# musyoku/chainer-speech-recognition

Hardware: AMD Instinct MI355X
Metric: utterances/sec (T=1000, 40x3 feat, |V|~3000) CTC train step (higher is better)
Workload: dtype bf16

## Files before the change

### chainer-speech-recognition_amd/asr/_lib.py

```python
import ctypes
import os

import torch

_HERE = os.path.dirname(os.path.abspath(__file__))
_ACT = os.environ.get("ASR_ACT", "").lower()
LIB_PATH = os.environ.get("ASR_HIP_LIB") or os.path.join(os.path.dirname(_HERE),
                                                        "libasr_hip_f16.so" if _ACT in ("f16", "fp16", "float16", "half") else "libasr_hip.so")

_lib = None


def act_dtype():
    return torch.float16 if lib().asr_act_dtype() else torch.bfloat16


def debug_flag(key, default):
    for item in os.environ.get("ASR_DEBUG", "").split(","):
        k, _, v = item.strip().partition("=")
        if k == key and v:
            return int(v)
    return default

c_void_p, c_int, c_float, c_size_t = ctypes.c_void_p, ctypes.c_int, ctypes.c_float, ctypes.c_size_t
c_double = ctypes.c_double
c_longlong = ctypes.c_longlong

SIGNATURES = {
    "asr_version": (c_int, []),
    "asr_act_dtype": (c_int, []),
    "asr_stream_delay": (c_int, [c_void_p, c_int]),
    "asr_occupy_cus": (c_int, [c_void_p, c_int, c_int, c_int]),
    "asr_stream_traffic": (c_int, [c_void_p, c_int, c_int, c_int, c_void_p, c_longlong]),
    "asr_ctc_workspace_bytes": (c_size_t, [c_int] * 5),
    "asr_ctc_forward": (c_int, [c_void_p] * 6 + [c_int] * 5 + [c_void_p] * 3 + [c_size_t]),
    "asr_ctc_forward_lse": (c_int, [c_void_p] * 6 + [c_int] * 5 + [c_void_p] * 3 + [c_size_t, c_void_p]),
    "asr_ctc_backward": (c_int, [c_void_p] * 3 + [c_int] * 5 + [c_void_p, c_int, c_float, c_void_p, c_void_p, c_size_t]),
    "asr_ctc_loss_grad": (c_int, [c_void_p] * 6 + [c_int] * 5 + [c_float] + [c_void_p] * 4 + [c_size_t]),
    "asr_ctc_nbest_workspace_bytes": (c_size_t, [c_int] * 5),
    "asr_ctc_nbest_forward": (c_int, [c_void_p] * 5 + [c_int] * 6 + [c_void_p, c_void_p, c_size_t]),
    "asr_ctc_nbest_backward": (c_int, [c_void_p] * 3 + [c_int] * 5 + [c_void_p] * 3 + [c_size_t]),
    "asr_gram_ctc_nbest_workspace_bytes": (c_size_t, [c_int] * 5),
    "asr_gram_ctc_nbest_forward": (c_int, [c_void_p] * 6 + [c_int] * 6 + [c_void_p, c_void_p, c_size_t]),
    "asr_gram_ctc_nbest_backward": (c_int, [c_void_p] * 3 + [c_int] * 5 + [c_void_p] * 3 + [c_size_t]),
    "asr_specgram": (c_int, [c_void_p, c_void_p, c_int, c_void_p, c_longlong] + [c_int] * 4 + [c_double, c_void_p, c_void_p, c_int,
                               c_void_p, c_void_p, c_int, c_void_p]),
    "asr_mel_bands_bytes": (c_size_t, []),
    "asr_mel_bands": (c_int, [c_void_p, c_void_p, c_int, c_int, c_void_p, c_size_t]),
    "asr_specgram_bands": (c_int, [c_void_p, c_void_p, c_int, c_void_p, c_longlong] + [c_int] * 4 + [c_double, c_void_p, c_void_p, c_int,
                                     c_void_p, c_void_p, c_int, c_void_p, c_void_p]),
    "asr_logmel": (c_int, [c_void_p] * 3 + [c_longlong, c_int, c_int, c_void_p]),
    "asr_deltas": (c_int, [c_void_p] * 3 + [c_int] * 4 + [c_void_p] * 3),
    "asr_batchnorm_stats": (c_int, [c_void_p, c_void_p, c_longlong, c_int, c_float, c_float] + [c_void_p] * 5),
    "asr_rsqrt_eps": (c_int, [c_void_p, c_void_p, c_float, c_void_p, c_int]),
    "asr_batchnorm_fwd": (c_int, [c_void_p] * 6 + [c_longlong, c_int, c_void_p]),
    "asr_batchnorm_bwd": (c_int, [c_void_p] * 6 + [c_longlong, c_int] + [c_void_p] * 4),
    "asr_cmn_pspec": (c_int, [c_void_p] * 3 + [c_int] * 3),
    "asr_add_white_noise": (c_int, [c_void_p] * 3 + [c_longlong, c_int, c_void_p, ctypes.c_ulonglong]),
    "asr_augment_specgram": (c_int, [c_void_p] * 5 + [c_int] * 4 + [c_void_p]),
    "asr_running_stats_update": (c_int, [c_void_p] * 3 + [c_int] * 3 + [c_longlong] + [c_void_p] * 4),
    "asr_normalize_bcmt": (c_int, [c_void_p] * 4 + [c_int] * 3),
    "asr_argmax_rows": (c_int, [c_void_p, c_void_p, c_int, c_int, c_int, c_void_p]),
    "asr_ctc_collapse": (c_int, [c_void_p] * 3 + [c_int] * 4 + [c_void_p] * 2),
    "asr_edit_distance": (c_int, [c_void_p, c_void_p, c_void_p, c_int, c_void_p, c_void_p, c_int, c_int, c_void_p]),
    "asr_edit_align_workspace_bytes": (c_size_t, [c_int] * 3),
    "asr_edit_align": (c_int, [c_void_p, c_void_p, c_void_p, c_int, c_void_p, c_void_p, c_int, c_int] + [c_void_p] * 4 + [c_size_t]),
    "asr_nbest_pairwise_distance": (c_int, [c_void_p] * 3 + [c_int] * 3 + [c_void_p]),
    "asr_nbest_consensus_workspace_bytes": (c_size_t, [c_int] * 3),
    "asr_nbest_consensus": (c_int, [c_void_p] * 5 + [c_int] * 3 + [c_void_p, c_void_p, c_size_t]),
    "asr_ctc_beam_workspace_bytes": (c_size_t, [c_int] * 5),
    "asr_ctc_beam_search": (c_int, [c_void_p] * 3 + [c_int] * 6 + [c_float, c_void_p, c_size_t] + [c_void_p] * 3),
    "asr_ngram_score": (c_int, [c_void_p] * 2 + [c_int, c_void_p, c_void_p] + [c_int] * 3 + [c_void_p] * 2 + [c_int] * 4 + [c_void_p] * 2),
    "asr_ctc_beam_lm_workspace_bytes": (c_size_t, [c_int] * 5),
    "asr_ctc_beam_search_lm": (c_int, [c_void_p] * 3 + [c_int] * 6 + [c_float, c_void_p, c_int, c_void_p, c_void_p] + [c_int] * 5
                               + [c_float, c_float, c_void_p, c_size_t] + [c_void_p] * 5),
    "asr_ctx_score": (c_int, [c_void_p] * 3 + [c_int] * 2 + [c_void_p] + [c_int] * 2 + [c_void_p] * 2 + [c_int] * 3 + [c_void_p] * 2),
    "asr_ctc_beam_bias_workspace_bytes": (c_size_t, [c_int] * 5),
    "asr_ctc_beam_search_bias": (c_int, [c_void_p] * 3 + [c_int] * 6 + [c_float, c_void_p, c_int, c_void_p, c_void_p] + [c_int] * 5
                                 + [c_float, c_float, c_void_p, c_size_t] + [c_void_p] * 7 + [c_int] * 2 + [c_void_p, c_int, c_void_p]),
    "asr_ctc_beam_stream_state_bytes": (c_size_t, [c_int] * 5),
    "asr_ctc_beam_stream_workspace_bytes": (c_size_t, [c_int] * 5),
    "asr_ctc_beam_stream_reset": (c_int, [c_void_p] * 2 + [c_size_t] + [c_int] * 6 + [c_void_p]),
    "asr_ctc_beam_stream_advance": (c_int, [c_void_p] * 3 + [c_int] * 6 + [c_float, c_void_p, c_int, c_void_p, c_void_p] + [c_int] * 3
                                    + [c_void_p] * 2 + [c_int] * 2 + [c_void_p, c_int, c_float, c_float, c_int, c_int]
                                    + [c_void_p, c_size_t] * 2),
    "asr_ctc_beam_stream_result": (c_int, [c_void_p] * 2 + [c_int, c_void_p, c_void_p] + [c_int] * 3 + [c_void_p] * 2 + [c_int] * 2
                                   + [c_void_p, c_int, c_float, c_float] + [c_int] * 6 + [c_void_p, c_size_t] + [c_void_p] * 7),
    "asr_gram_ctc_beam_workspace_bytes": (c_size_t, [c_int] * 5),
    "asr_gram_ctc_beam_search": (c_int, [c_void_p] * 3 + [c_int] * 6 + [c_float, c_void_p, c_void_p, c_size_t] + [c_void_p] * 3),
    "asr_gram_ctc_beam_lm_workspace_bytes": (c_size_t, [c_int] * 5),
    "asr_gram_ctc_beam_search_lm": (c_int, [c_void_p] * 3 + [c_int] * 6 + [c_float, c_void_p, c_void_p, c_int, c_void_p, c_void_p]
                                    + [c_int] * 5 + [c_float, c_float, c_void_p, c_size_t] + [c_void_p] * 5),
    "asr_gram_ctc_beam_stream_state_bytes": (c_size_t, [c_int] * 4),
    "asr_gram_ctc_beam_stream_workspace_bytes": (c_size_t, [c_int] * 5),
    "asr_gram_ctc_beam_stream_reset": (c_int, [c_void_p] * 2 + [c_size_t] + [c_int] * 4 + [c_void_p]),
    "asr_gram_ctc_beam_stream_advance": (c_int, [c_void_p] * 3 + [c_int] * 6 + [c_float, c_void_p, c_void_p, c_int, c_void_p, c_void_p]
                                         + [c_int] * 4 + [c_float, c_float, c_int, c_int] + [c_void_p, c_size_t] * 2),
    "asr_gram_ctc_beam_stream_result": (c_int, [c_void_p] * 2 + [c_int, c_void_p, c_void_p] + [c_int] * 5 + [c_float, c_float]
                                        + [c_int] * 5 + [c_void_p, c_size_t] + [c_void_p] * 6),
    "asr_gram_ctc_beam_bias_workspace_bytes": (c_size_t, [c_int] * 5),
    "asr_gram_ctc_beam_search_bias": (c_int, [c_void_p] * 3 + [c_int] * 6 + [c_float, c_void_p, c_void_p, c_int, c_void_p, c_void_p]
                                      + [c_int] * 5 + [c_float, c_float, c_void_p, c_size_t] + [c_void_p] * 7 + [c_int] * 2
                                      + [c_void_p, c_int, c_void_p]),
    "asr_gram_ctc_beam_bias_stream_state_bytes": (c_size_t, [c_int] * 5),
    "asr_gram_ctc_beam_bias_stream_reset": (c_int, [c_void_p] * 2 + [c_size_t] + [c_int] * 5 + [c_void_p]),
    "asr_gram_ctc_beam_bias_stream_advance": (c_int, [c_void_p] * 3 + [c_int] * 6 + [c_float, c_void_p, c_void_p, c_int, c_void_p,
                                                      c_void_p] + [c_int] * 4 + [c_void_p] * 2 + [c_int] * 2 + [c_void_p, c_int]
                                              + [c_float, c_float, c_int, c_int] + [c_void_p, c_size_t] * 2),
    "asr_gram_ctc_beam_bias_stream_result": (c_int, [c_void_p] * 2 + [c_int, c_void_p, c_void_p] + [c_int] * 5 + [c_void_p] * 2
                                             + [c_int] * 2 + [c_void_p, c_int] + [c_float, c_float] + [c_int] * 5
                                             + [c_void_p, c_size_t] + [c_void_p] * 7),
    "asr_ctc_align_workspace_bytes": (c_size_t, [c_int] * 5),
    "asr_ctc_align": (c_int, [c_void_p] * 6 + [c_int] * 5 + [c_void_p] * 9 + [c_size_t]),
    "asr_kws_workspace_bytes": (c_size_t, [c_int] * 3),
    "asr_kws_state_bytes": (c_size_t, [c_int] * 3),
    "asr_kws_state_reset": (c_int, [c_void_p] * 2 + [c_int] * 3 + [c_void_p]),
    "asr_kws_detect": (c_int, [c_void_p] * 3 + [c_int] * 4 + [c_void_p, c_int, c_void_p, c_void_p, c_int, c_int] + [c_void_p] * 5
                       + [c_size_t]),
    "asr_kws_hits": (c_int, [c_void_p] * 5 + [c_int] * 4 + [c_float] + [c_void_p] * 5),
# ... 147 lines not shown
```

### chainer-speech-recognition_amd/csrc/ctc.hip

```cpp
#include "common.hpp"
#include "ctc_ws.hpp"
#include "ctc_lattice.hpp"
#include "ctc_sweep.hpp"
#include "../../include/asr_hip.h"

namespace asr {
namespace ctc {

__global__ __launch_bounds__(256) void rows_kernel(const float* __restrict__ xs, const int* __restrict__ x_len,
                                                   const int* __restrict__ path_label, int T, int B, int V, int Sp,
                                                   float* __restrict__ lse_out, float* __restrict__ lp, const float* __restrict__ lse_in) {
    __shared__ float scratch[32];
    if (lse_in) {
        const int row = blockIdx.x * 4 + (int)(threadIdx.x >> 6), lane = threadIdx.x & 63;
        if (row >= T * B) return;
        const int t = row / B, b = row - t * B;
        const int xl = x_len ? min(x_len[b], T) : T;
        if (t >= xl) return;
        const float* x = xs + (size_t)row * V;
        const float lse = lse_in[row];
        if (lane == 0) lse_out[row] = lse;
        const int* pl = path_label + (size_t)b * Sp;
        float* out = lp + ((size_t)b * T + t) * Sp;
        for (int s = lane; s < Sp; s += 64) {
            const int l = pl[s];
            out[s] = l >= 0 ? x[l] - lse : -INFINITY;
        }
        return;
    }
    const int row = blockIdx.x;
    const int t = row / B, b = row - t * B;
    const int xl = x_len ? min(x_len[b], T) : T;
    if (t >= xl) return;
    const float* x = xs + (size_t)row * V;
    float m = -INFINITY;
    const bool vec = ((V & 3) == 0) && ((((uintptr_t)x) & 15) == 0);
    if (vec) {
        const float4* x4 = reinterpret_cast<const float4*>(x);
        for (int i = threadIdx.x; i < (V >> 2); i += blockDim.x) {
            const float4 v = x4[i];
            m = fmaxf(m, fmaxf(fmaxf(v.x, v.y), fmaxf(v.z, v.w)));
        }
    } else {
        for (int i = threadIdx.x; i < V; i += blockDim.x) m = fmaxf(m, x[i]);
    }
    m = block_max(m, scratch);
    float sum = 0.f;
    if (vec) {
        const float4* x4 = reinterpret_cast<const float4*>(x);
        for (int i = threadIdx.x; i < (V >> 2); i += blockDim.x) {
            const float4 v = x4[i];
            sum += __expf(v.x - m) + __expf(v.y - m) + __expf(v.z - m) + __expf(v.w - m);
        }
    } else {
        for (int i = threadIdx.x; i < V; i += blockDim.x) sum += __expf(x[i] - m);
    }
    sum = block_sum(sum, scratch);
    const float lse = m + __logf(sum);
    if (threadIdx.x == 0) lse_out[row] = lse;
    const int* pl = path_label + (size_t)b * Sp;
    float* out = lp + ((size_t)b * T + t) * Sp;
    for (int s = threadIdx.x; s < Sp; s += blockDim.x) {
        const int l = pl[s];
        out[s] = l >= 0 ? x[l] - lse : -INFINITY;
    }
}

constexpr int kOccChunk = 8192;

__global__ __launch_bounds__(256) void grad_kernel(const float* __restrict__ xs, const int* __restrict__ x_len,
                                                   const int* __restrict__ path_label,
                                                   const int* __restrict__ path_len, const float* __restrict__ lse_in,
                                                   const double* __restrict__ alpha, const double* __restrict__ beta,
                                                   const double* __restrict__ total, const float* __restrict__ gy,
                                                   int gy_per_utt, float scale, int T, int B, int V, int Sp,
                                                   float* __restrict__ grad) {
    extern __shared__ __attribute__((aligned(16))) char smem[];
    float* occ = reinterpret_cast<float*>(smem);
    const int row = blockIdx.x;
    const int t = row / B, b = row - t * B;
    const int xl = x_len ? min(x_len[b], T) : T;
    float* g = grad + (size_t)row * V;
    const bool vec = ((V & 3) == 0) && ((((uintptr_t)g) & 15) == 0) && ((((uintptr_t)(xs + (size_t)row * V)) & 15) == 0);
    if (t >= xl) {
        if (vec) {
            float4* g4 = reinterpret_cast<float4*>(g);
            for (int i = threadIdx.x; i < (V >> 2); i += blockDim.x) g4[i] = make_float4(0.f, 0.f, 0.f, 0.f);
        } else {
            for (int i = threadIdx.x; i < V; i += blockDim.x) g[i] = 0.f;
        }
        return;
    }
    const float* x = xs + (size_t)row * V;
    const float lse = lse_in[row];
    const double tot = total[b];
    float sc = scale;
    if (gy) sc *= gy_per_utt ? gy[b] : gy[0];
    const int S = path_len[b];
    const int* pl = path_label + (size_t)b * Sp;
    const double* al = alpha + ((size_t)b * T + t) * Sp;
    const double* be = beta + ((size_t)b * T + t) * Sp;
    for (int v0 = 0; v0 < V; v0 += kOccChunk) {
        const int vn = min(kOccChunk, V - v0);
        for (int i = threadIdx.x; i < vn; i += blockDim.x) occ[i] = 0.f;
        __syncthreads();
        if (tot != -INFINITY) {
            for (int s = threadIdx.x; s < S; s += blockDim.x) {
                const int l = pl[s];
                if (l >= v0 && l < v0 + vn) {
                    const double e = al[s] + be[s] - tot;
                    if (e > -80.0) atomicAdd(&occ[l - v0], expf((float)e));
                }
            }
        }
        __syncthreads();
        if (vec) {
            const float4* x4 = reinterpret_cast<const float4*>(x + v0);
            const float4* o4 = reinterpret_cast<const float4*>(occ);
            float4* g4 = reinterpret_cast<float4*>(g + v0);
            for (int i = threadIdx.x; i < (vn >> 2); i += blockDim.x) {
                const float4 xv = x4[i];
                const float4 ov = o4[i];
                float4 r;
                r.x = (__expf(xv.x - lse) - ov.x) * sc;
                r.y = (__expf(xv.y - lse) - ov.y) * sc;
                r.z = (__expf(xv.z - lse) - ov.z) * sc;
                r.w = (__expf(xv.w - lse) - ov.w) * sc;
                g4[i] = r;
            }
        } else {
            for (int i = threadIdx.x; i < vn; i += blockDim.x) g[v0 + i] = (__expf(x[v0 + i] - lse) - occ[i]) * sc;
        }
        __syncthreads();
    }
}

__global__ void mean_kernel(const float* __restrict__ loss, int B, float* __restrict__ out) {
    __shared__ float scratch[32];
    float s = 0.f;
    for (int i = threadIdx.x; i < B; i += blockDim.x) s += loss[i];
    s = block_sum(s, scratch);
    if (threadIdx.x == 0) out[0] = s / (float)B;
}

}
}

using namespace asr;
using namespace asr::ctc;

extern "C" size_t asr_ctc_workspace_bytes(int T, int B, int V, int Lmax, int gram) {
    (void)V;
    if (T <= 0 || B <= 0 || Lmax <= 0) return 0;
    return carve(nullptr, T, B, Lmax, gram).bytes;
}

extern "C" int asr_ctc_forward_lse(void* stream_, const float* xs, const int32_t* label_unigram,
                                   const int32_t* label_bigram, const int32_t* x_len, const int32_t* l_len, int T, int B,
                                   int V, int Lmax, int blank, float* loss_per_utt, float* loss_mean, void* workspace,
                                   size_t workspace_bytes, const float* row_lse) {
    if (!xs || !label_unigram || !loss_per_utt || !workspace) return ASR_ERR_BAD_ARG;
    if (T <= 0 || B <= 0 || V <= 0 || Lmax <= 0 || blank < 0 || blank >= V) return ASR_ERR_BAD_ARG;
    const int gram = label_bigram != nullptr;
    Workspace w = carve(workspace, T, B, Lmax, gram);
    if (workspace_bytes < w.bytes) return ASR_ERR_WORKSPACE;
    const int Sp = path_pad(Lmax, gram);
    const size_t lds = sizeof(double) * 2 * (Sp + 16) + sizeof(int) * (Sp + 8);
    if (lds > 150 * 1024) return ASR_ERR_UNSUPPORTED;
    hipStream_t stream = (hipStream_t)stream_;
    if (gram)
        hipLaunchKernelGGL(prep_kernel<true>, dim3(B), dim3(256), 0, stream, label_unigram, label_bigram, l_len, Lmax, Sp,
                           V, blank, w.path_label, w.path_mask, w.path_len);
    else
        hipLaunchKernelGGL(prep_kernel<false>, dim3(B), dim3(256), 0, stream, label_unigram, label_bigram, l_len, Lmax,
                           Sp, V, blank, w.path_label, w.path_mask, w.path_len);
    ASR_LAUNCH_CHECK();
    hipLaunchKernelGGL(rows_kernel, dim3(row_lse ? (T * B + 3) / 4 : T * B), dim3(256), 0, stream, xs, x_len, w.path_label, T, B, V, Sp, w.lse, w.lp, row_lse);
    ASR_LAUNCH_CHECK();
    const int threads = Sp < 1024 ? Sp : 1024;
    if (gram) {
        if (lds > 48 * 1024)
            (void)hipFuncSetAttribute((const void*)lattice_kernel<7>, hipFuncAttributeMaxDynamicSharedMemorySize, (int)lds);
        hipLaunchKernelGGL(lattice_kernel<7>, dim3(B, 2), dim3(threads), lds, stream, w.lp, x_len, w.path_label,
                           w.path_mask, w.path_len, T, B, Sp, w.alpha, w.beta, w.total, loss_per_utt);
    } else {
        if (lds > 48 * 1024)
            (void)hipFuncSetAttribute((const void*)lattice_kernel<3>, hipFuncAttributeMaxDynamicSharedMemorySize, (int)lds);
        hipLaunchKernelGGL(lattice_kernel<3>, dim3(B, 2), dim3(threads), lds, stream, w.lp, x_len, w.path_label,
                           w.path_mask, w.path_len, T, B, Sp, w.alpha, w.beta, w.total, loss_per_utt);
    }
    ASR_LAUNCH_CHECK();
    if (loss_mean) {
        hipLaunchKernelGGL(mean_kernel, dim3(1), dim3(256), 0, stream, loss_per_utt, B, loss_mean);
        ASR_LAUNCH_CHECK();
    }
    return ASR_OK;
}

extern "C" int asr_ctc_forward(void* stream_, const float* xs, const int32_t* label_unigram,
                               const int32_t* label_bigram, const int32_t* x_len, const int32_t* l_len, int T, int B,
                               int V, int Lmax, int blank, float* loss_per_utt, float* loss_mean, void* workspace,
                               size_t workspace_bytes) {
    return asr_ctc_forward_lse(stream_, xs, label_unigram, label_bigram, x_len, l_len, T, B, V, Lmax, blank, loss_per_utt, loss_mean,
                               workspace, workspace_bytes, nullptr);
}

extern "C" int asr_ctc_backward(void* stream_, const float* xs, const int32_t* x_len, int T, int B, int V, int Lmax,
                                int gram, const float* gy, int gy_per_utt, float scale, float* grad,
                                const void* workspace, size_t workspace_bytes) {
    if (!xs || !grad || !workspace) return ASR_ERR_BAD_ARG;
    if (T <= 0 || B <= 0 || V <= 0 || Lmax <= 0) return ASR_ERR_BAD_ARG;
    Workspace w = carve(const_cast<void*>(workspace), T, B, Lmax, gram);
    if (workspace_bytes < w.bytes) return ASR_ERR_WORKSPACE;
    const int Sp = path_pad(Lmax, gram);
    const size_t lds = sizeof(float) * (size_t)(V < kOccChunk ? (int)align_up(V, 4) : kOccChunk);
    hipStream_t stream = (hipStream_t)stream_;
    hipLaunchKernelGGL(grad_kernel, dim3(T * B), dim3(256), lds, stream, xs, x_len, w.path_label, w.path_len, w.lse,
                       w.alpha, w.beta, w.total, gy, gy_per_utt, scale, T, B, V, Sp, grad);
    ASR_LAUNCH_CHECK();
    return ASR_OK;
}

extern "C" int asr_ctc_loss_grad(void* stream, const float* xs, const int32_t* label_unigram,
                                 const int32_t* label_bigram, const int32_t* x_len, const int32_t* l_len, int T, int B,
                                 int V, int Lmax, int blank, float scale, float* loss_per_utt, float* loss_mean,
                                 float* grad, void* workspace, size_t workspace_bytes) {
    int rc = asr_ctc_forward(stream, xs, label_unigram, label_bigram, x_len, l_len, T, B, V, Lmax, blank, loss_per_utt,
                             loss_mean, workspace, workspace_bytes);
    if (rc != ASR_OK) return rc;
    return asr_ctc_backward(stream, xs, x_len, T, B, V, Lmax, label_bigram != nullptr, nullptr, 0, scale, grad,
                            workspace, workspace_bytes);
}
```

### chainer-speech-recognition_amd/csrc/ctc_sweep.hpp

```cpp
#pragma once
#include "common.hpp"
#include "ctc_lattice.hpp"

namespace asr {
namespace ctc {

template <int NK>
__device__ __forceinline__ double lse_masked(const double* v, int mask) {
    float f[NK];
#pragma unroll
    for (int j = 0; j < NK; ++j) f[j] = (mask & (1 << j)) ? (float)v[j] : -INFINITY;
    float m32 = -1e30f;
#pragma unroll
    for (int j = 0; j < NK; ++j) m32 = __builtin_fmaxf(m32, f[j]);
    const double m = (double)m32;
    float acc = 0.f;
#pragma unroll
    for (int j = 0; j < NK; ++j) {
        const float e = __expf((float)(v[j] - m));
        acc += (mask & (1 << j)) ? e : 0.f;
    }
    return m + (double)(__builtin_amdgcn_logf(acc) * 0.69314718f);
}

template <int NK>
__global__ __launch_bounds__(1024) void lattice_kernel(const float* __restrict__ lp, const int* __restrict__ x_len,
                                                       const int* __restrict__ path_label,
                                                       const int* __restrict__ path_mask,
                                                       const int* __restrict__ path_len, int T, int B, int Sp,
                                                       double* __restrict__ alpha, double* __restrict__ beta,
                                                       double* __restrict__ total, float* __restrict__ loss) {
    extern __shared__ __attribute__((aligned(16))) char smem[];
    double* buf0 = reinterpret_cast<double*>(smem);
    double* buf1 = buf0 + (Sp + 16);
    int* mask_s = reinterpret_cast<int*>(buf1 + (Sp + 16));
    const int b = blockIdx.x;
    const bool backward = blockIdx.y == 1;
    const int xl = x_len ? min(x_len[b], T) : T;
    const int S = path_len[b];
    const float* lpb = lp + (size_t)b * T * Sp;
    double* outb = (backward ? beta : alpha) + (size_t)b * T * Sp;
    const int* pm = path_mask + (size_t)b * Sp;
    const int* pl = path_label + (size_t)b * Sp;

    for (int i = threadIdx.x; i < Sp + 16; i += blockDim.x) {
        buf0[i] = -INFINITY;
        buf1[i] = -INFINITY;
    }
    for (int i = threadIdx.x; i < Sp + 8; i += blockDim.x) mask_s[i] = i < Sp ? pm[i] : 0;
    __syncthreads();
    double* prev = buf0 + 8;
    double* cur = buf1 + 8;

    if (xl <= 0) {
        if (!backward && threadIdx.x == 0) { total[b] = -INFINITY; loss[b] = 1e10f; }
        return;
    }

    const bool one_node = (int)blockDim.x >= Sp;
    constexpr int PF = 4;
    if (!backward && one_node) {
        if (threadIdx.x == 0) prev[0] = 0.0;
        __syncthreads();
        const int sidx = threadIdx.x;
        const int mk = mask_s[sidx];
        float lq[PF];
#pragma unroll
        for (int j = 0; j < PF; ++j) lq[j] = lpb[(size_t)min(j, xl - 1) * Sp + sidx];
        int t0 = 0;
        for (; t0 + PF <= xl; t0 += PF) {
#pragma unroll
            for (int j = 0; j < PF; ++j) {
                const int t = t0 + j;
                double v[NK];
#pragma unroll
                for (int q = 0; q < NK; ++q) v[q] = prev[sidx - koff<NK>(q)];
                const double a = lse_masked<NK>(v, mk) + (double)lq[j];
                cur[sidx] = a;
                outb[(size_t)t * Sp + sidx] = a;
                lq[j] = lpb[(size_t)min(t + PF, xl - 1) * Sp + sidx];
                ASR_LDS_BARRIER();
                double* tmp = prev; prev = cur; cur = tmp;
            }
        }
#pragma unroll
        for (int j = 0; j < PF - 1; ++j) {
            const int t = t0 + j;
            if (t < xl) {
                double v[NK];
#pragma unroll
                for (int q = 0; q < NK; ++q) v[q] = prev[sidx - koff<NK>(q)];
                const double a = lse_masked<NK>(v, mk) + (double)lq[j];
                cur[sidx] = a;
                outb[(size_t)t * Sp + sidx] = a;
                ASR_LDS_BARRIER();
                double* tmp = prev; prev = cur; cur = tmp;
            }
        }
        if (threadIdx.x == 0) {
            double v[3] = {-INFINITY, -INFINITY, -INFINITY};
            v[0] = prev[S - 1];
            if (S >= 2) v[1] = prev[S - 2];
            if (NK != 3 && S >= 3) v[2] = prev[S - 3];
            const double tot = lse_masked<3>(v, 7);
            total[b] = tot;
            loss[b] = tot == -INFINITY ? 1e10f : (float)(-tot);
        }
    } else if (backward && one_node) {
        const int sidx = threadIdx.x;
        bool fin;
        if (NK == 3) fin = (sidx == S - 1) || (sidx == S - 2 && S >= 2);
        else fin = (sidx == S - 1) || (S >= 3 && (sidx == S - 2 || sidx == S - 3));
        fin = fin && pl[sidx] >= 0;
        const double bt0 = fin ? 0.0 : -INFINITY;
        outb[(size_t)(xl - 1) * Sp + sidx] = bt0;
        prev[sidx] = bt0 + (double)lpb[(size_t)(xl - 1) * Sp + sidx];
        int mkd = 0;
#pragma unroll
        for (int q = 0; q < NK; ++q) mkd |= ((mask_s[sidx + koff<NK>(q)] >> q) & 1) << q;
        __syncthreads();
        float lq[PF];
#pragma unroll
        for (int j = 0; j < PF; ++j) lq[j] = lpb[(size_t)max(xl - 2 - j, 0) * Sp + sidx];
        int t0 = xl - 2;
        for (; t0 - (PF - 1) >= 0; t0 -= PF) {
#pragma unroll
            for (int j = 0; j < PF; ++j) {
                const int t = t0 - j;
                double v[NK];
#pragma unroll
                for (int q = 0; q < NK; ++q) v[q] = prev[sidx + koff<NK>(q)];
                const double bt = lse_masked<NK>(v, mkd);
                outb[(size_t)t * Sp + sidx] = bt;
                cur[sidx] = bt + (double)lq[j];
                lq[j] = lpb[(size_t)max(t - PF, 0) * Sp + sidx];
                ASR_LDS_BARRIER();
                double* tmp = prev; prev = cur; cur = tmp;
            }
        }
#pragma unroll
        for (int j = 0; j < PF - 1; ++j) {
            const int t = t0 - j;
            if (t >= 0) {
                double v[NK];
#pragma unroll
                for (int q = 0; q < NK; ++q) v[q] = prev[sidx + koff<NK>(q)];
                const double bt = lse_masked<NK>(v, mkd);
                outb[(size_t)t * Sp + sidx] = bt;
                cur[sidx] = bt + (double)lq[j];
                ASR_LDS_BARRIER();
                double* tmp = prev; prev = cur; cur = tmp;
            }
        }
    } else if (!backward) {
        if (threadIdx.x == 0) prev[0] = 0.0;
        __syncthreads();
        for (int t = 0; t < xl; ++t) {
            const float* lpt = lpb + (size_t)t * Sp;
            double* ot = outb + (size_t)t * Sp;
            for (int s = threadIdx.x; s < Sp; s += blockDim.x) {
                const int mk = mask_s[s];
                double v[NK];
#pragma unroll
                for (int j = 0; j < NK; ++j) v[j] = prev[s - koff<NK>(j)];
                double a = lse_masked<NK>(v, mk);
                a += (double)lpt[s];
                cur[s] = a;
                ot[s] = a;
            }
            __syncthreads();
            double* tmp = prev; prev = cur; cur = tmp;
        }
        if (threadIdx.x == 0) {
            double v[3] = {-INFINITY, -INFINITY, -INFINITY};
            v[0] = prev[S - 1];
            if (S >= 2) v[1] = prev[S - 2];
            if (NK != 3 && S >= 3) v[2] = prev[S - 3];
            const double tot = lse_masked<3>(v, 7);
            total[b] = tot;
            loss[b] = tot == -INFINITY ? 1e10f : (float)(-tot);
        }
    } else {
        for (int s = threadIdx.x; s < Sp; s += blockDim.x) {
            bool fin;
            if (NK == 3) fin = (s == S - 1) || (s == S - 2 && S >= 2);
            else fin = (s == S - 1) || (S >= 3 && (s == S - 2 || s == S - 3));
            fin = fin && pl[s] >= 0;
            const double bt = fin ? 0.0 : -INFINITY;
            outb[(size_t)(xl - 1) * Sp + s] = bt;
            prev[s] = bt + (double)lpb[(size_t)(xl - 1) * Sp + s];
        }
        __syncthreads();
        for (int t = xl - 2; t >= 0; --t) {
            const float* lpt = lpb + (size_t)t * Sp;
            double* ot = outb + (size_t)t * Sp;
            for (int s = threadIdx.x; s < Sp; s += blockDim.x) {
                double v[NK];
                int mk = 0;
#pragma unroll
                for (int j = 0; j < NK; ++j) {
                    const int k = koff<NK>(j);
                    v[j] = prev[s + k];
                    mk |= ((mask_s[s + k] >> j) & 1) << j;
                }
                const double bt = lse_masked<NK>(v, mk);
                ot[s] = bt;
                cur[s] = bt + (double)lpt[s];
            }
            __syncthreads();
            double* tmp = prev; prev = cur; cur = tmp;
        }
    }
}

}
}
```

### include/asr_hip.h

```cpp
#ifndef ASR_HIP_H
#define ASR_HIP_H
#include <stddef.h>
#include <stdint.h>
#ifdef __cplusplus
extern "C" {
#endif

int asr_version(void);
int asr_act_dtype(void);
int asr_stream_delay(void* stream, int microseconds);
int asr_occupy_cus(void* stream, int microseconds, int lds_bytes, int blocks);
int asr_stream_traffic(void* stream, int microseconds, int lds_bytes, int blocks, void* buf, long long bytes);

size_t asr_ctc_workspace_bytes(int T, int B, int V, int Lmax, int gram);
int asr_ctc_forward(void* stream, const float* xs, const int32_t* label_unigram, const int32_t* label_bigram,
                    const int32_t* x_len, const int32_t* l_len, int T, int B, int V, int Lmax, int blank,
                    float* loss_per_utt, float* loss_mean, void* workspace, size_t workspace_bytes);
int asr_ctc_forward_lse(void* stream, const float* xs, const int32_t* label_unigram, const int32_t* label_bigram,
                        const int32_t* x_len, const int32_t* l_len, int T, int B, int V, int Lmax, int blank, float* loss_per_utt,
                        float* loss_mean, void* workspace, size_t workspace_bytes, const float* row_lse);
int asr_ctc_backward(void* stream, const float* xs, const int32_t* x_len, int T, int B, int V, int Lmax, int gram,
                     const float* gy, int gy_per_utt, float scale, float* grad, const void* workspace,
                     size_t workspace_bytes);
int asr_ctc_loss_grad(void* stream, const float* xs, const int32_t* label_unigram, const int32_t* label_bigram,
                      const int32_t* x_len, const int32_t* l_len, int T, int B, int V, int Lmax, int blank, float scale,
                      float* loss_per_utt, float* loss_mean, float* grad, void* workspace, size_t workspace_bytes);
size_t asr_ctc_nbest_workspace_bytes(int T, int B, int V, int N, int Lmax);
int asr_ctc_nbest_forward(void* stream, const float* xs, const int32_t* hyp, const int32_t* hyp_len, const int32_t* x_len, int T,
                          int B, int V, int N, int Lmax, int blank, float* logp, void* workspace, size_t workspace_bytes);
int asr_ctc_nbest_backward(void* stream, const float* xs, const int32_t* x_len, int T, int B, int V, int N, int Lmax,
                           const float* gy, float* grad, const void* workspace, size_t workspace_bytes);
size_t asr_gram_ctc_nbest_workspace_bytes(int T, int B, int V, int N, int Lmax);
int asr_gram_ctc_nbest_forward(void* stream, const float* xs, const int32_t* hyp, const int32_t* hyp_len, const int32_t* x_len,
                               const int32_t* gram, int T, int B, int V, int N, int Lmax, int blank, float* logp, void* workspace,
                               size_t workspace_bytes);
int asr_gram_ctc_nbest_backward(void* stream, const float* xs, const int32_t* x_len, int T, int B, int V, int N, int Lmax,
                                const float* gy, float* grad, const void* workspace, size_t workspace_bytes);

int asr_specgram(void* stream, const void* signals, int sig_is_f32, const int32_t* lengths, long long sig_pitch, int B,
                 int frame_len, int frame_step, int nfft, double preemph, const float* window, const int32_t* nframes,
                 int Fmax, float* pspec_out, const float* fbank, int nfilt, float* logmel_out);
size_t asr_mel_bands_bytes(void);
int asr_mel_bands(void* stream, const float* fbank, int nfilt, int nbins, void* table, size_t table_bytes);
int asr_specgram_bands(void* stream, const void* signals, int sig_is_f32, const int32_t* lengths, long long sig_pitch, int B,
                       int frame_len, int frame_step, int nfft, double preemph, const float* window, const int32_t* nframes,
                       int Fmax, float* pspec_out, const float* fbank, int nfilt, float* logmel_out, const void* bands);
int asr_logmel(void* stream, const float* pspec, const float* fbank, long long F, int nbins, int nfilt, float* out);
int asr_deltas(void* stream, const float* logmel, const int32_t* nframes, int B, int Fmax, int nfilt, int Tmax,
               const float* mean, const float* stdv, float* out);

int asr_cmn_pspec(void* stream, float* pspec, const int32_t* nframes, int B, int Fmax, int nbins);
int asr_add_white_noise(void* stream, float* signals, const int32_t* lengths, long long pitch, int B, const float* gain,
                        unsigned long long seed);
int asr_augment_specgram(void* stream, const float* pspec_in, const int32_t* nframes_out, const double* speed,
                         const double* ratio, int B, int Fmax_in, int Fmax_out, int nbins, float* pspec_out);
int asr_running_stats_update(void* stream, const float* x, const int32_t* lengths, int B, int CM, int T,
                             long long total_before, double* mean, double* nvar, float* mean32, float* std32);
int asr_normalize_bcmt(void* stream, float* x, const float* mean, const float* stdv, int B, int CM, int T);

int asr_argmax_rows(void* stream, const float* logits, int T, int B, int V, int32_t* ids);
int asr_ctc_collapse(void* stream, const int32_t* ids, const int32_t* lengths, int B, int T, int blank, int merge_repeats,
                     int32_t* out, int32_t* out_len);
int asr_edit_distance(void* stream, const int32_t* ref, const int32_t* ref_len, int ref_pitch, const int32_t* hyp,
                      const int32_t* hyp_len, int hyp_pitch, int pairs, int32_t* dist);
size_t asr_edit_align_workspace_bytes(int pairs, int ref_pitch, int hyp_pitch);
int asr_edit_align(void* stream, const int32_t* ref, const int32_t* ref_len, int ref_pitch, const int32_t* hyp,
                   const int32_t* hyp_len, int hyp_pitch, int pairs, int32_t* counts, int32_t* ref_to_hyp, int32_t* hyp_to_ref,
                   void* workspace, size_t workspace_bytes);
int asr_nbest_pairwise_distance(void* stream, const int32_t* ids, const int32_t* lens, int B, int N, int pitch, int32_t* dist);
size_t asr_nbest_consensus_workspace_bytes(int B, int N, int pitch);
int asr_nbest_consensus(void* stream, const int32_t* ids, const int32_t* lens, const int32_t* pivot, const float* post, int B,
                        int N, int pitch, float* conf, void* workspace, size_t workspace_bytes);
size_t asr_ctc_beam_workspace_bytes(int T, int B, int V, int beam_width, int top_k);
int asr_ctc_beam_search(void* stream, const float* logits, const int32_t* lengths, int T, int B, int V, int blank, int beam_width,
                        int top_k, float min_logp, void* workspace, size_t workspace_bytes, int32_t* out_ids, int32_t* out_len,
                        float* out_score);
size_t asr_ctc_align_workspace_bytes(int T, int B, int V, int Lmax, int gram);
int asr_ctc_align(void* stream, const float* xs, const int32_t* label_unigram, const int32_t* label_bigram, const int32_t* x_len,
                  const int32_t* l_len, int T, int B, int V, int Lmax, int blank, int32_t* frame_ids, int32_t* tok_ids,
                  int32_t* tok_pos, int32_t* tok_start, int32_t* tok_end, float* tok_logp, int32_t* n_tok, float* score,
                  void* workspace, size_t workspace_bytes);
size_t asr_kws_workspace_bytes(int T, int B, int U);
size_t asr_kws_state_bytes(int B, int K, int Lmax);
int asr_kws_state_reset(void* stream, void* state, int B, int K, int Lmax, const int32_t* mask);
int asr_kws_detect(void* stream, const float* logits, const int32_t* lengths, int T, int B, int V, int blank, const int32_t* uniq,
                   int U, const int32_t* node_tok, const int32_t* kw_len, int K, int Lmax, void* state, float* det,
                   int32_t* det_start, float* fill, void* workspace, size_t workspace_bytes);
int asr_kws_hits(void* stream, const float* det, const int32_t* det_start, const float* fill, const int32_t* lengths, int B, int K,
                 int T, int max_hits, float min_score, int32_t* hit_start, int32_t* hit_end, float* hit_score, float* hit_logp,
                 int32_t* n_hits);
size_t asr_gram_kws_state_bytes(int B, int K, int Lmax);
int asr_gram_kws_state_reset(void* stream, void* state, int B, int K, int Lmax, const int32_t* mask);
int asr_gram_kws_detect(void* stream, const float* logits, const int32_t* lengths, int T, int B, int V, int blank,
                        const int32_t* uniq, int U, const int32_t* node_uni, const int32_t* node_big, const int32_t* kw_len, int K,
                        int Lmax, void* state, float* det, int32_t* det_start, float* fill, void* workspace,
                        size_t workspace_bytes);
int asr_ngram_score(void* stream, const float* uni, int vlm, const int32_t* keys, const float* vals, int slots, int max_probe,
                    int order, const int32_t* ids, const int32_t* lengths, int N, int Lmax, int bos, int eos, float* out_tok,
                    float* out_sum);
size_t asr_ctc_beam_lm_workspace_bytes(int T, int B, int V, int beam_width, int top_k);
int asr_ctc_beam_search_lm(void* stream, const float* logits, const int32_t* lengths, int T, int B, int V, int blank,
                           int beam_width, int top_k, float min_logp, const float* uni, int vlm, const int32_t* keys,
                           const float* vals, int slots, int max_probe, int order, int bos, int eos, float alpha, float beta,
// ... 251 lines not shown
```

Measured before the change: 2462.

## Fuse emission gather into CTC lattice kernel, skipping the lp table

Adds a direct-source path where the forward/backward lattice kernel gathers x[label] and the row LSE straight from the activations, instead of reading a precomputed per-path log-prob table. When the LSE is already available, the rows_kernel launch and the T*B*Sp table write and read are skipped, and the LSE copy into the workspace happens inside the lattice kernel. The lattice kernel now does scattered gathers from a V-wide row on every step, so it uses a deeper prefetch depth plus explicit waitcnt and register pinning to hide that latency. asr_ctc_forward_lse defaults to the direct path whenever Sp <= 1024.

```diff
diff --git a/chainer-speech-recognition_amd/asr/_lib.py b/chainer-speech-recognition_amd/asr/_lib.py
--- a/chainer-speech-recognition_amd/asr/_lib.py
+++ b/chainer-speech-recognition_amd/asr/_lib.py
@@ -35,6 +35,7 @@
     "asr_ctc_workspace_bytes": (c_size_t, [c_int] * 5),
     "asr_ctc_forward": (c_int, [c_void_p] * 6 + [c_int] * 5 + [c_void_p] * 3 + [c_size_t]),
     "asr_ctc_forward_lse": (c_int, [c_void_p] * 6 + [c_int] * 5 + [c_void_p] * 3 + [c_size_t, c_void_p]),
+    "asr_ctc_forward_src": (c_int, [c_void_p] * 6 + [c_int] * 5 + [c_void_p] * 3 + [c_size_t, c_void_p, c_int]),
     "asr_ctc_backward": (c_int, [c_void_p] * 3 + [c_int] * 5 + [c_void_p, c_int, c_float, c_void_p, c_void_p, c_size_t]),
     "asr_ctc_loss_grad": (c_int, [c_void_p] * 6 + [c_int] * 5 + [c_float] + [c_void_p] * 4 + [c_size_t]),
     "asr_ctc_nbest_workspace_bytes": (c_size_t, [c_int] * 5),
diff --git a/chainer-speech-recognition_amd/csrc/ctc.hip b/chainer-speech-recognition_amd/csrc/ctc.hip
--- a/chainer-speech-recognition_amd/csrc/ctc.hip
+++ b/chainer-speech-recognition_amd/csrc/ctc.hip
@@ -58,6 +58,7 @@
     sum = block_sum(sum, scratch);
     const float lse = m + __logf(sum);
     if (threadIdx.x == 0) lse_out[row] = lse;
+    if (!lp) return;
     const int* pl = path_label + (size_t)b * Sp;
     float* out = lp + ((size_t)b * T + t) * Sp;
     for (int s = threadIdx.x; s < Sp; s += blockDim.x) {
@@ -155,10 +156,28 @@
     return carve(nullptr, T, B, Lmax, gram).bytes;
 }
 
-extern "C" int asr_ctc_forward_lse(void* stream_, const float* xs, const int32_t* label_unigram,
+template <int NK>
+static void launch_lattice(hipStream_t stream, bool direct, const float* xs, const float* row_lse, const Workspace& w,
+                           const int32_t* x_len, int T, int B, int V, int Sp, int threads, size_t lds, float* loss_per_utt) {
+    if (direct) {
+        if (lds > 48 * 1024)
+            (void)hipFuncSetAttribute((const void*)lattice_direct_kernel<NK>, hipFuncAttributeMaxDynamicSharedMemorySize, (int)lds);
+        hipLaunchKernelGGL(lattice_direct_kernel<NK>, dim3(B, 2), dim3(threads), lds, stream, xs, row_lse ? row_lse : w.lse, V,
+                           x_len, w.path_label, w.path_mask, w.path_len, T, B, Sp, w.alpha, w.beta, w.total, loss_per_utt,
+                           row_lse ? w.lse : nullptr);
+    } else {
+        if (lds > 48 * 1024)
+            (void)hipFuncSetAttribute((const void*)lattice_kernel<NK>, hipFuncAttributeMaxDynamicSharedMemorySize, (int)lds);
+        hipLaunchKernelGGL(lattice_kernel<NK>, dim3(B, 2), dim3(threads), lds, stream, w.lp, x_len, w.path_label, w.path_mask,
+                           w.path_len, T, B, Sp, w.alpha, w.beta, w.total, loss_per_utt);
+    }
+}
+
+extern "C" int asr_ctc_forward_src(void* stream_, const float* xs, const int32_t* label_unigram,
                                    const int32_t* label_bigram, const int32_t* x_len, const int32_t* l_len, int T, int B,
                                    int V, int Lmax, int blank, float* loss_per_utt, float* loss_mean, void* workspace,
-                                   size_t workspace_bytes, const float* row_lse) {
+                                   size_t workspace_bytes, const float* row_lse, int source) {
+    if (source != ASR_CTC_SOURCE_TABLE && source != ASR_CTC_SOURCE_DIRECT) return ASR_ERR_BAD_ARG;
     if (!xs || !label_unigram || !loss_per_utt || !workspace) return ASR_ERR_BAD_ARG;
     if (T <= 0 || B <= 0 || V <= 0 || Lmax <= 0 || blank < 0 || blank >= V) return ASR_ERR_BAD_ARG;
     const int gram = label_bigram != nullptr;
@@ -175,26 +194,31 @@
         hipLaunchKernelGGL(prep_kernel<false>, dim3(B), dim3(256), 0, stream, label_unigram, label_bigram, l_len, Lmax,
                            Sp, V, blank, w.path_label, w.path_mask, w.path_len);
     ASR_LAUNCH_CHECK();
-    hipLaunchKernelGGL(rows_kernel, dim3(row_lse ? (T * B + 3) / 4 : T * B), dim3(256), 0, stream, xs, x_len, w.path_label, T, B, V, Sp, w.lse, w.lp, row_lse);
-    ASR_LAUNCH_CHECK();
+    const bool direct = source == ASR_CTC_SOURCE_DIRECT && Sp <= 1024;
+    if (!direct) {
+        hipLaunchKernelGGL(rows_kernel, dim3(row_lse ? (T * B + 3) / 4 : T * B), dim3(256), 0, stream, xs, x_len, w.path_label, T, B, V, Sp, w.lse, w.lp, row_lse);
+        ASR_LAUNCH_CHECK();
+    } else if (!row_lse) {
+        hipLaunchKernelGGL(rows_kernel, dim3(T * B), dim3(256), 0, stream, xs, x_len, w.path_label, T, B, V, Sp, w.lse, (float*)nullptr, (const float*)nullptr);
+        ASR_LAUNCH_CHECK();
+    }
     const int threads = Sp < 1024 ? Sp : 1024;
-    if (gram) {
-        if (lds > 48 * 1024)
-            (void)hipFuncSetAttribute((const void*)lattice_kernel<7>, hipFuncAttributeMaxDynamicSharedMemorySize, (int)lds);
-        hipLaunchKernelGGL(lattice_kernel<7>, dim3(B, 2), dim3(threads), lds, stream, w.lp, x_len, w.path_label,
-                           w.path_mask, w.path_len, T, B, Sp, w.alpha, w.beta, w.total, loss_per_utt);
-    } else {
-        if (lds > 48 * 1024)
-            (void)hipFuncSetAttribute((const void*)lattice_kernel<3>, hipFuncAttributeMaxDynamicSharedMemorySize, (int)lds);
-        hipLaunchKernelGGL(lattice_kernel<3>, dim3(B, 2), dim3(threads), lds, stream, w.lp, x_len, w.path_label,
-                           w.path_mask, w.path_len, T, B, Sp, w.alpha, w.beta, w.total, loss_per_utt);
-    }
+    if (gram) launch_lattice<7>(stream, direct, xs, row_lse, w, x_len, T, B, V, Sp, threads, lds, loss_per_utt);
+    else launch_lattice<3>(stream, direct, xs, row_lse, w, x_len, T, B, V, Sp, threads, lds, loss_per_utt);
     ASR_LAUNCH_CHECK();
     if (loss_mean) {
         hipLaunchKernelGGL(mean_kernel, dim3(1), dim3(256), 0, stream, loss_per_utt, B, loss_mean);
         ASR_LAUNCH_CHECK();
     }
     return ASR_OK;
+}
+
+extern "C" int asr_ctc_forward_lse(void* stream_, const float* xs, const int32_t* label_unigram,
+                                   const int32_t* label_bigram, const int32_t* x_len, const int32_t* l_len, int T, int B,
+                                   int V, int Lmax, int blank, float* loss_per_utt, float* loss_mean, void* workspace,
+                                   size_t workspace_bytes, const float* row_lse) {
+    return asr_ctc_forward_src(stream_, xs, label_unigram, label_bigram, x_len, l_len, T, B, V, Lmax, blank, loss_per_utt, loss_mean,
+                               workspace, workspace_bytes, row_lse, ASR_CTC_SOURCE_DIRECT);
 }
 
 extern "C" int asr_ctc_forward(void* stream_, const float* xs, const int32_t* label_unigram,
diff --git a/chainer-speech-recognition_amd/csrc/ctc_sweep.hpp b/chainer-speech-recognition_amd/csrc/ctc_sweep.hpp
--- a/chainer-speech-recognition_amd/csrc/ctc_sweep.hpp
+++ b/chainer-speech-recognition_amd/csrc/ctc_sweep.hpp
@@ -23,13 +23,63 @@
     return m + (double)(__builtin_amdgcn_logf(acc) * 0.69314718f);
 }
 
-template <int NK>
-__global__ __launch_bounds__(1024) void lattice_kernel(const float* __restrict__ lp, const int* __restrict__ x_len,
-                                                       const int* __restrict__ path_label,
-                                                       const int* __restrict__ path_mask,
-                                                       const int* __restrict__ path_len, int T, int B, int Sp,
-                                                       double* __restrict__ alpha, double* __restrict__ beta,
-                                                       double* __restrict__ total, float* __restrict__ loss) {
+struct TableSource {
+    const float* lp;
+    static constexpr int kPF = 4;
+    typedef float Raw;
+    struct Bound {
+        const float* lpb;
+        int Sp;
+        __device__ __forceinline__ Raw fetch(int t, int s, int) const { return lpb[(size_t)t * Sp + s]; }
+        static __device__ __forceinline__ float value(Raw r, int) { return r; }
+        static __device__ __forceinline__ void settle() {}
+        static __device__ __forceinline__ void pin(Raw&) {}
+    };
+    __device__ __forceinline__ Bound bind(int b, int T, int, int Sp) const { return Bound{lp + (size_t)b * T * Sp, Sp}; }
+};
+
+#ifndef ASR_CTC_DIRECT_PF
+#define ASR_CTC_DIRECT_PF 8
+#endif
+struct DirectSource {
+    const float* xs;
+    const float* lse;
+    int V;
+    static constexpr int kPF = ASR_CTC_DIRECT_PF;
+    struct Raw { float x, lse; };
+    struct Bound {
+        const float* xb;
+        const float* lb;
+        size_t BV;
+        int B;
+        unsigned vz;
+        __device__ __forceinline__ Raw fetch(int t, int, int label) const {
+            Raw r;
+            r.x = (xb + (size_t)t * BV)[(unsigned)max(label, 0)];
+            r.lse = (lb + (size_t)t * B)[vz];
+            return r;
+        }
+        static __device__ __forceinline__ float value(Raw r, int label) {
+            float e = label >= 0 ? r.x - r.lse : -INFINITY;
+            asm("" : "+v"(e));
+            return e;
+        }
+        static __device__ __forceinline__ void settle() { __builtin_amdgcn_s_waitcnt(0x0f70); }
+        static __device__ __forceinline__ void pin(Raw& r) { asm volatile("" : "+v"(r.x), "+v"(r.lse)); }
+    };
+    __device__ __forceinline__ Bound bind(int b, int, int B, int) const {
+        unsigned vz;
+        asm volatile("v_mov_b32 %0, 0" : "=v"(vz));
+        return Bound{xs + (size_t)b * V, lse + b, (size_t)B * V, B, vz};
+    }
+};
+
+template <int NK, class Src>
+__device__ __forceinline__ void lattice_body(const Src src, const int* __restrict__ x_len, const int* __restrict__ path_label,
+                                             const int* __restrict__ path_mask, const int* __restrict__ path_len, int T, int B,
+                                             int Sp, double* __restrict__ alpha, double* __restrict__ beta,
+                                             double* __restrict__ total, float* __restrict__ loss, const float* lse_in,
+                                             float* lse_copy) {
     extern __shared__ __attribute__((aligned(16))) char smem[];
     double* buf0 = reinterpret_cast<double*>(smem);
     double* buf1 = buf0 + (Sp + 16);
@@ -38,7 +88,7 @@
     const bool backward = blockIdx.y == 1;
     const int xl = x_len ? min(x_len[b], T) : T;
     const int S = path_len[b];
-    const float* lpb = lp + (size_t)b * T * Sp;
+    const typename Src::Bound em = src.bind(b, T, B, Sp);
     double* outb = (backward ? beta : alpha) + (size_t)b * T * Sp;
     const int* pm = path_mask + (size_t)b * Sp;
     const int* pl = path_label + (size_t)b * Sp;
@@ -58,27 +108,32 @@
     }
 
     const bool one_node = (int)blockDim.x >= Sp;
-    constexpr int PF = 4;
+    constexpr int PF = Src::kPF;
     if (!backward && one_node) {
         if (threadIdx.x == 0) prev[0] = 0.0;
         __syncthreads();
         const int sidx = threadIdx.x;
         const int mk = mask_s[sidx];
-        float lq[PF];
-#pragma unroll
-        for (int j = 0; j < PF; ++j) lq[j] = lpb[(size_t)min(j, xl - 1) * Sp + sidx];
+        const int lab = pl[sidx];
+        typename Src::Raw lq[PF];
+#pragma unroll
+        for (int j = 0; j < PF; ++j) lq[j] = em.fetch(min(j, xl - 1), sidx, lab);
+        if (lse_copy)
+            for (int t = threadIdx.x; t < xl; t += blockDim.x) lse_copy[(size_t)t * B + b] = lse_in[(size_t)t * B + b];
+        Src::Bound::settle();
         int t0 = 0;
         for (; t0 + PF <= xl; t0 += PF) {
 #pragma unroll
             for (int j = 0; j < PF; ++j) {
                 const int t = t0 + j;
+                Src::Bound::pin(lq[j]);
                 double v[NK];
 #pragma unroll
                 for (int q = 0; q < NK; ++q) v[q] = prev[sidx - koff<NK>(q)];
-                const double a = lse_masked<NK>(v, mk) + (double)lq[j];
+                const double a = lse_masked<NK>(v, mk) + (double)Src::Bound::value(lq[j], lab);
                 cur[sidx] = a;
                 outb[(size_t)t * Sp + sidx] = a;
-                lq[j] = lpb[(size_t)min(t + PF, xl - 1) * Sp + sidx];
+                lq[j] = em.fetch(min(t + PF, xl - 1), sidx, lab);
                 ASR_LDS_BARRIER();
                 double* tmp = prev; prev = cur; cur = tmp;
             }
@@ -90,7 +145,7 @@
                 double v[NK];
 #pragma unroll
                 for (int q = 0; q < NK; ++q) v[q] = prev[sidx - koff<NK>(q)];
-                const double a = lse_masked<NK>(v, mk) + (double)lq[j];
+                const double a = lse_masked<NK>(v, mk) + (double)Src::Bound::value(lq[j], lab);
                 cur[sidx] = a;
                 outb[(size_t)t * Sp + sidx] = a;
                 ASR_LDS_BARRIER();
@@ -111,29 +166,32 @@
         bool fin;
         if (NK == 3) fin = (sidx == S - 1) || (sidx == S - 2 && S >= 2);
         else fin = (sidx == S - 1) || (S >= 3 && (sidx == S - 2 || sidx == S - 3));
-        fin = fin && pl[sidx] >= 0;
+        const int lab = pl[sidx];
+        fin = fin && lab >= 0;
         const double bt0 = fin ? 0.0 : -INFINITY;
         outb[(size_t)(xl - 1) * Sp + sidx] = bt0;
-        prev[sidx] = bt0 + (double)lpb[(size_t)(xl - 1) * Sp + sidx];
+        prev[sidx] = bt0 + (double)Src::Bound::value(em.fetch(xl - 1, sidx, lab), lab);
         int mkd = 0;
 #pragma unroll
         for (int q = 0; q < NK; ++q) mkd |= ((mask_s[sidx + koff<NK>(q)] >> q) & 1) << q;
         __syncthreads();
-        float lq[PF];
-#pragma unroll
-        for (int j = 0; j < PF; ++j) lq[j] = lpb[(size_t)max(xl - 2 - j, 0) * Sp + sidx];
+        typename Src::Raw lq[PF];
+#pragma unroll
+        for (int j = 0; j < PF; ++j) lq[j] = em.fetch(max(xl - 2 - j, 0), sidx, lab);
+        Src::Bound::settle();
         int t0 = xl - 2;
         for (; t0 - (PF - 1) >= 0; t0 -= PF) {
 #pragma unroll
             for (int j = 0; j < PF; ++j) {
                 const int t = t0 - j;
+                Src::Bound::pin(lq[j]);
                 double v[NK];
 #pragma unroll
                 for (int q = 0; q < NK; ++q) v[q] = prev[sidx + koff<NK>(q)];
                 const double bt = lse_masked<NK>(v, mkd);
                 outb[(size_t)t * Sp + sidx] = bt;
-                cur[sidx] = bt + (double)lq[j];
-                lq[j] = lpb[(size_t)max(t - PF, 0) * Sp + sidx];
+                cur[sidx] = bt + (double)Src::Bound::value(lq[j], lab);
+                lq[j] = em.fetch(max(t - PF, 0), sidx, lab);
                 ASR_LDS_BARRIER();
                 double* tmp = prev; prev = cur; cur = tmp;
             }
@@ -147,7 +205,7 @@
                 for (int q = 0; q < NK; ++q) v[q] = prev[sidx + koff<NK>(q)];
                 const double bt = lse_masked<NK>(v, mkd);
                 outb[(size_t)t * Sp + sidx] = bt;
-                cur[sidx] = bt + (double)lq[j];
+                cur[sidx] = bt + (double)Src::Bound::value(lq[j], lab);
                 ASR_LDS_BARRIER();
                 double* tmp = prev; prev = cur; cur = tmp;
             }
@@ -156,7 +214,6 @@
         if (threadIdx.x == 0) prev[0] = 0.0;
         __syncthreads();
         for (int t = 0; t < xl; ++t) {
-            const float* lpt = lpb + (size_t)t * Sp;
             double* ot = outb + (size_t)t * Sp;
             for (int s = threadIdx.x; s < Sp; s += blockDim.x) {
                 const int mk = mask_s[s];
@@ -164,7 +221,7 @@
 #pragma unroll
                 for (int j = 0; j < NK; ++j) v[j] = prev[s - koff<NK>(j)];
                 double a = lse_masked<NK>(v, mk);
-                a += (double)lpt[s];
+                a += (double)Src::Bound::value(em.fetch(t, s, pl[s]), pl[s]);
                 cur[s] = a;
                 ot[s] = a;
             }
@@ -188,11 +245,10 @@
             fin = fin && pl[s] >= 0;
             const double bt = fin ? 0.0 : -INFINITY;
             outb[(size_t)(xl - 1) * Sp + s] = bt;
-            prev[s] = bt + (double)lpb[(size_t)(xl - 1) * Sp + s];
+            prev[s] = bt + (double)Src::Bound::value(em.fetch(xl - 1, s, pl[s]), pl[s]);
         }
         __syncthreads();
         for (int t = xl - 2; t >= 0; --t) {
-            const float* lpt = lpb + (size_t)t * Sp;
             double* ot = outb + (size_t)t * Sp;
             for (int s = threadIdx.x; s < Sp; s += blockDim.x) {
                 double v[NK];
@@ -205,7 +261,7 @@
                 }
                 const double bt = lse_masked<NK>(v, mk);
                 ot[s] = bt;
-                cur[s] = bt + (double)lpt[s];
+                cur[s] = bt + (double)Src::Bound::value(em.fetch(t, s, pl[s]), pl[s]);
             }
             __syncthreads();
             double* tmp = prev; prev = cur; cur = tmp;
@@ -213,5 +269,29 @@
     }
 }
 
-}
-}
+template <int NK>
+__global__ __launch_bounds__(1024) void lattice_kernel(const float* __restrict__ lp, const int* __restrict__ x_len,
+                                                       const int* __restrict__ path_label,
+                                                       const int* __restrict__ path_mask,
+                                                       const int* __restrict__ path_len, int T, int B, int Sp,
+                                                       double* __restrict__ alpha, double* __restrict__ beta,
+                                                       double* __restrict__ total, float* __restrict__ loss) {
+    lattice_body<NK>(TableSource{lp}, x_len, path_label, path_mask, path_len, T, B, Sp, alpha, beta, total, loss, nullptr, nullptr);
+}
+
+template <int NK>
+__global__ __launch_bounds__(1024) void lattice_direct_kernel(const float* __restrict__ xs, const float* lse, int V,
+                                                              const int* __restrict__ x_len,
+                                                              const int* __restrict__ path_label,
+                                                              const int* __restrict__ path_mask,
+                                                              const int* __restrict__ path_len, int T, int B, int Sp,
+                                                              double* __restrict__ alpha, double* __restrict__ beta,
+                                                              double* __restrict__ total, float* __restrict__ loss,
+                                                              float* lse_copy) {
+    lattice_body<NK>(DirectSource{xs, lse, V}, x_len, path_label, path_mask, path_len, T, B, Sp, alpha, beta, total, loss, lse,
+                     lse_copy);
+}
+
+
+}
+}
diff --git a/include/asr_hip.h b/include/asr_hip.h
--- a/include/asr_hip.h
+++ b/include/asr_hip.h
@@ -19,6 +19,11 @@
 int asr_ctc_forward_lse(void* stream, const float* xs, const int32_t* label_unigram, const int32_t* label_bigram,
                         const int32_t* x_len, const int32_t* l_len, int T, int B, int V, int Lmax, int blank, float* loss_per_utt,
                         float* loss_mean, void* workspace, size_t workspace_bytes, const float* row_lse);
+#define ASR_CTC_SOURCE_TABLE 0
+#define ASR_CTC_SOURCE_DIRECT 1
+int asr_ctc_forward_src(void* stream, const float* xs, const int32_t* label_unigram, const int32_t* label_bigram,
+                        const int32_t* x_len, const int32_t* l_len, int T, int B, int V, int Lmax, int blank, float* loss_per_utt,
+                        float* loss_mean, void* workspace, size_t workspace_bytes, const float* row_lse, int source);
 int asr_ctc_backward(void* stream, const float* xs, const int32_t* x_len, int T, int B, int V, int Lmax, int gram,
                      const float* gy, int gy_per_utt, float scale, float* grad, const void* workspace,
                      size_t workspace_bytes);
```

Result: no change. 2459 (-0.1%).
